# zhengyk19/vit-rpe-rope

Measured on AMD Instinct MI355X. Metric: train images/sec, CIFAR-10 ViT d=192 L=6 H=6, higher is better.
Workload: dtype bf16; 1 GPU; CIFAR-10-shaped 32x32 patch4 ViT d=192 L=6 H=6, --pos_encoding rope-axial theta=100, bf16, full train step (fwd+CE+bwd+AdamW), random-init weights; per_gpu_batch=512, global_batch=512, parallelism=dp1, hip_graph=True

## Files before the change

### include/vitpe_debug.h

```cpp
#ifndef VITPE_DEBUG_H
#define VITPE_DEBUG_H
#include "vitpe.h"
#ifdef __cplusplus
extern "C" {
#endif

int vitpe_selftest_mma(int dtype, const void* A, const void* Bt, const void* Brow, float* C_row,
                       float* C_tr, vitpe_stream_t stream);

int vitpe_debug_wgrad_census(int dtype, const vitpe_wgrad_problem* problems, int nprob, unsigned long long* census,
                             vitpe_stream_t stream);
int vitpe_debug_attn_census(const void* xn, const void* wqkv, void* out, const float* cos, const float* sin,
                            int B, unsigned long long* census, vitpe_stream_t stream);
int vitpe_debug_attn32_census(const void* xn, const void* wqkv_wide, void* out, const float* cos, const float* sin,
                              int B, unsigned long long* census, vitpe_stream_t stream);
int vitpe_debug_tail2_census(const void* attn_out, const void* x_in, const void* Wp_packed, const float* bp,
                             const float* gamma, const float* beta, void* x_mid, float* mean2, float* rstd2,
                             void* xn_out, const void* W1_packed, const float* b1, const void* W2_packed,
                             const float* b2, void* gp_out, void* h_out, void* out, float* mean_out, float* rstd_out,
                             int M, int HID, unsigned long long* census, vitpe_stream_t stream);
int vitpe_debug_set_gemm2d_mt(int mt);
int vitpe_debug_set_wgrad_wide(int on);
int vitpe_debug_read_bw(const void* src, long long bytes, int depth, int workgroups, unsigned* sink, vitpe_stream_t stream);
#ifdef __cplusplus
}
#endif
#endif
```

### vit-rpe-rope_amd/csrc/attn.hip

```cpp
#include "attn_common.h"
#include <stdlib.h>
#include <type_traits>

namespace vitpe {

template <typename T, typename C, int KM, int NTH = 384>
VITPE_DEV void stage_tokens(const AttnArgs& a, int b, T* xs, T* hbuf, int hbuf_elems, float* s_tab, float* s_coef,
                            int tid, int nthreads, bool stage_tables) {
  constexpr int CHN = CH<T>::n;
  constexpr int DCH = C::LDX / CHN;
  constexpr int D = C::DD;
  const int N = C::ntok(a);
  const T* xg = reinterpret_cast<const T*>(a.xn) + (size_t)b * N * D;
  const Chunk16 zero = {0u, 0u, 0u, 0u};
  constexpr int TOTAL = C::NP * DCH;
  constexpr int ITERS = (TOTAL + NTH - 1) / NTH;
  Chunk16 v[ITERS];
#pragma unroll
  for (int it = 0; it < ITERS; ++it) {
    const int q = tid + it * nthreads, row = q / DCH, cc = q % DCH;
    v[it] = zero;
    if (q < TOTAL && row < N && cc * CHN < D) v[it] = *reinterpret_cast<const Chunk16*>(xg + (size_t)row * D + cc * CHN);
  }
  if (a.ln_gamma != nullptr) {
// ... 477 lines not shown
    Frag<T> xf[KS];
#pragma unroll
    for (int ks = 0; ks < KS; ++ks) xf[ks] = ld_frag(xrow + 16 * tt * C::LDX + 32 * ks);
    __builtin_amdgcn_sched_barrier(0);
    f32x4 acc[NT] = {z4, z4};
#pragma unroll
    for (int ks = 0; ks < KS; ++ks)
#pragma unroll
      for (int nt = 0; nt < NT; ++nt) mma(w[nt][ks], xf[ks], acc[nt]);
    __builtin_amdgcn_sched_barrier(0);
    if (KM == KM_ROPE && rope) {
      f32x4 cv, sv;
      cs_vec(16 * tt + c, 4 * g, cv, sv);
      const f32x4 x1 = acc[0], x2 = acc[1];
      acc[0] = x1 * cv - x2 * sv;
      acc[1] = x1 * sv + x2 * cv;
    }
    dst = acc_to_frag<T>(acc[0] * sc, acc[1] * sc);
    asm volatile("" : "+v"(dst.v));
  };
  Frag<T> e0, e1;
#pragma unroll
  for (int t = 0; t < 8; ++t) {
    e0.v[t] = (bf16)((t < 4 && 4 * g + t == c) ? 1.0f : 0.0f);
    e1.v[t] = (bf16)((t >= 4 && 4 * g + t - 4 == c) ? 1.0f : 0.0f);
  }
  auto transpose_pair = [&](const Frag<T>& fa, const Frag<T>* fb, Frag<T>& d0, Frag<T>& d1) {
    f32x4 a0 = z4, a1 = z4, b0 = z4, b1 = z4;
    mma(fa, e0, a0);
    mma(fa, e1, a1);
    if (fb != nullptr) { mma(*fb, e0, b0); mma(*fb, e1, b1); }
    d0 = acc_to_frag<T>(a0, b0);
    d1 = acc_to_frag<T>(a1, b1);
  };

  const float qsc = a.scale * LOG2E;
  Frag<T> vkf[MT], kf[MT];
#pragma unroll
  for (int tt = 0; tt < MT; ++tt) proj_sw(tt, false, 1.0f, vkf[tt]);
  wload(w, 1);
  __builtin_amdgcn_sched_barrier(0);
#pragma unroll
  for (int tt = 0; tt < MT; ++tt) proj_sw(tt, true, 1.0f, kf[tt]);
  wload(w, 0);
  __builtin_amdgcn_sched_barrier(0);
#pragma unroll
  for (int tt = 0; tt < MT; ++tt) {
    Frag<T> qf;
    proj_sw(tt, true, qsc, qf);
    *reinterpret_cast<bf16x8*>(qsw + tt * FRAG) = qf.v;
  }
  __syncthreads();
  if (!live) return;
  {
    const T* dog = reinterpret_cast<const T*>(a.dout) + (size_t)b * N * D + h * HD;
    Frag<T> df[MT];
#pragma unroll
    for (int tt = 0; tt < MT; ++tt) {
      const int tok = 16 * tt + c;
      bf16x4 lo = {(bf16)0.f, (bf16)0.f, (bf16)0.f, (bf16)0.f}, hi = lo;
      if (tok < N) {
        lo = *reinterpret_cast<const bf16x4*>(dog + (size_t)tok * D + 4 * g);
        hi = *reinterpret_cast<const bf16x4*>(dog + (size_t)tok * D + 16 + 4 * g);
      }
      df[tt].v = __builtin_shufflevector(lo, hi, 0, 1, 2, 3, 4, 5, 6, 7);
    }
#pragma unroll
    for (int tt = 0; tt < MT; ++tt) *reinterpret_cast<bf16x8*>(dsw + tt * FRAG) = df[tt].v;
  }
  auto qf_load = [&](int tt) { Frag<T> f; f.v = *reinterpret_cast<const bf16x8*>(qsw + tt * FRAG); return f; };
  auto dof_load = [&](int tt) { Frag<T> f; f.v = *reinterpret_cast<const bf16x8*>(dsw + tt * FRAG); return f; };
  Frag<T> ktf[NT][SC];
#pragma unroll
  for (int scx = 0; scx < SC; ++scx)
    transpose_pair(kf[2 * scx], (2 * scx + 1 < MT) ? &kf[(2 * scx + 1 < MT) ? 2 * scx + 1 : 0] : nullptr, ktf[0][scx], ktf[1][scx]);

  T* const dqg = reinterpret_cast<T*>(a.out) + (size_t)b * N * 3 * D + h * HD;
  auto store_pair = [&](T* rowp, const f32x4& o0, const f32x4& o1, bool ok) {
    uint32_t lo[2], hi[2];
#pragma unroll
    for (int w2 = 0; w2 < 2; ++w2) {
      bf16x2 pa, pb;
      pa[0] = (bf16)o0[2 * w2]; pa[1] = (bf16)o0[2 * w2 + 1];
      pb[0] = (bf16)o1[2 * w2]; pb[1] = (bf16)o1[2 * w2 + 1];
      const auto r = __builtin_amdgcn_permlane16_swap(__builtin_bit_cast(uint32_t, pa), __builtin_bit_cast(uint32_t, pb), false, false);
      lo[w2] = r[0]; hi[w2] = r[1];
    }
    const int f0 = 16 * (g & 1) + 8 * (g >> 1);
    if (ok) *reinterpret_cast<Chunk16*>(rowp + f0) = (Chunk16){lo[0], lo[1], hi[0], hi[1]};
  };

  float cacc[PDEG + 1];
#pragma unroll
  for (int k = 0; k <= PDEG; ++k) cacc[k] = 0.f;
#pragma unroll
  for (int it = 0; it < MT; ++it) {
    __builtin_amdgcn_sched_barrier(0);
    const int i = 16 * it + c;
    const Frag<T> dof = dof_load(it), qfi = qf_load(it);
    f32x4 s[MT], dp[MT];
    float m = -1e30f;
    typedef __attribute__((ext_vector_type(4))) unsigned u32x4;
    const unsigned xyi = (KM == KM_POLY) ? reinterpret_cast<const unsigned*>(s_coef + C::H * C::PBLD)[i] : 0u;
    const float* const ptab = s_coef + (a.coeff_per_head ? h : 0) * C::PBLD;
    const bool qcls = (it == 0) && (c == 0);
#pragma unroll
    for (int jt = 0; jt < MT; ++jt) {
      s[jt] = z4;
      mma(kf[jt], qfi, s[jt]);
      dp[jt] = z4;
      mma(vkf[jt], dof, dp[jt]);
      const u32x4 xyj = (KM == KM_POLY) ? *reinterpret_cast<const u32x4*>(s_coef + C::H * C::PBLD + 16 * jt + 4 * g) : (u32x4){0u, 0u, 0u, 0u};
#pragma unroll
      for (int r = 0; r < 4; ++r) {
        const int j = 16 * jt + 4 * g + r;
        float v = s[jt][r];
        if (KM == KM_RELATIVE) v += pe_bias2<C, KM>(a, s_tab, s_coef, h, i, j, N);
        if (KM == KM_POLY) {
          const float bv = ptab[__builtin_amdgcn_sad_u8(xyi, xyj[r], 0u)];
          const bool cls = qcls || (jt == 0 && r == 0 && g == 0);
          v += cls ? 0.f : bv;
        }
        if (jt == MT - 1) v = (j < N) ? v : -1e30f;
        s[jt][r] = v;
        m = fmaxf(m, v);
      }
    }
    m = xg_max(m);
    float l = 0.f;
#pragma unroll
    for (int jt = 0; jt < MT; ++jt)
#pragma unroll
      for (int r = 0; r < 4; ++r) { const float p = __builtin_amdgcn_exp2f(s[jt][r] - m); s[jt][r] = p; l += p; }
    l = xg_sum(l);
    const float inv = __builtin_amdgcn_rcpf(l);
    float dl = 0.f;
#pragma unroll
    for (int jt = 0; jt < MT; ++jt)
#pragma unroll
      for (int r = 0; r < 4; ++r) { s[jt][r] *= inv; dl += s[jt][r] * dp[jt][r]; }
    dl = xg_sum(dl);
    if (g == 0) { lse_w[i] = m + __builtin_amdgcn_logf(l); del_w[i] = dl; }
    const bool qvalid = (it < MT - 1) || (i < N);
    float tacc[PDEG + 1];
#pragma unroll
    for (int k = 0; k <= PDEG; ++k) tacc[k] = 0.f;
#pragma unroll
    for (int jt = 0; jt < MT; ++jt) {
      if (KM == KM_POLY) __builtin_amdgcn_sched_barrier(0);
      const u32x4 xyj = (KM == KM_POLY) ? *reinterpret_cast<const u32x4*>(s_coef + C::H * C::PBLD + 16 * jt + 4 * g) : (u32x4){0u, 0u, 0u, 0u};
#pragma unroll
      for (int r = 0; r < 4; ++r) {
        const int j = 16 * jt + 4 * g + r;
        const bool valid = qvalid && ((jt < MT - 1) || (j < N));
        const float ds = valid ? s[jt][r] * (dp[jt][r] - dl) : 0.f;
        dp[jt][r] = ds;
        if (KM == KM_POLY) {
          const float dsk = (jt == 0 && r == 0) ? (g == 0 ? 0.f : ds) : ds;
          const float x = (float)__builtin_amdgcn_sad_u8(xyi, xyj[r], 0u);
          float pw = x;
          tacc[0] += dsk;
#pragma unroll
          for (int k = 1; k <= PDEG; ++k) { tacc[k] = fmaf(dsk, pw, tacc[k]); if (k < PDEG) pw *= x; }
        }
      }
    }
    if (KM == KM_POLY) {
      const float qm = (it == 0 && c == 0) ? 0.f : 1.f;
#pragma unroll
      for (int k = 0; k <= PDEG; ++k) {
        cacc[k] = fmaf(qm, tacc[k], cacc[k]);
        asm volatile("" : "+v"(cacc[k]));
      }
    }
    if (KM == KM_RELATIVE) {
#pragma unroll
      for (int jt = 0; jt < MT; ++jt) {
        float d0, d1;
        tile_diag_sums(dp[jt], lane, d0, d1);
        const int idx0 = 16 * (it - jt) + c + N - 1;
        if (g == 0) {
          if (idx0 >= 0 && idx0 <= 2 * N - 2) atomicAdd(&dtab_i[h * C::TABLD + idx0], d0);
          if (c >= 1 && idx0 - 16 >= 0 && idx0 - 16 <= 2 * N - 2) atomicAdd(&dtab_i[h * C::TABLD + idx0 - 16], d1);
        }
      }
    }
    f32x4 dqa[NT] = {z4, z4};
#pragma unroll
    for (int scx = 0; scx < SC; ++scx) {
      const Frag<T> bs = acc_to_frag<T>(dp[2 * scx], (2 * scx + 1 < MT) ? dp[(2 * scx + 1 < MT) ? 2 * scx + 1 : 0] : z4);
#pragma unroll
      for (int dt = 0; dt < NT; ++dt) mma(ktf[dt][scx], bs, dqa[dt]);
    }
    if (mixed) {
      const bool tok_ok = i >= 1 && i < N;
      f32x4 dph;
#pragma unroll
      for (int r = 0; r < 4; ++r) dph[r] = dqa[1][r] * (float)qfi.v[r] - dqa[0][r] * (float)qfi.v[4 + r];
      mixed_freq_grad_tile(dfreq_i, dph, i, tok_ok, 16 * it, h, C::H, P, a.grid, HD / 2, 4 * g, LN2, lane);
    }
    if (KM == KM_ROPE) {
      f32x4 cv, sv;
      cs_vec(min(i, C::NP - 1), 4 * g, cv, sv);
      const f32x4 d1 = dqa[0], d2 = dqa[1];
      dqa[0] = d1 * cv + d2 * sv;
      dqa[1] = d2 * cv - d1 * sv;
    }
    store_pair(dqg + (size_t)i * 3 * D, dqa[0] * a.scale, dqa[1] * a.scale, qvalid);
  }

  if (KM == KM_POLY) {
#pragma unroll
    for (int k = 0; k <= PDEG; ++k)
      if (k <= a.degree) {
        const float t = wave_sum(cacc[k]);
        if (lane == 0) atomicAdd(&dcoef_i[(a.coeff_per_head ? h : 0) * (C::MAXDEG + 1) + k], t);
      }
  }
  Frag<T> qtf[NT][SC], dotf[NT][SC];
  __builtin_amdgcn_sched_barrier(0);
#pragma unroll
  for (int scx = 0; scx < SC; ++scx) {
    const bool two = 2 * scx + 1 < MT;
    const Frag<T> qa = qf_load(2 * scx), qb = qf_load(two ? 2 * scx + 1 : 0);
    transpose_pair(qa, two ? &qb : nullptr, qtf[0][scx], qtf[1][scx]);
    const Frag<T> da = dof_load(2 * scx), db = dof_load(two ? 2 * scx + 1 : 0);
    transpose_pair(da, two ? &db : nullptr, dotf[0][scx], dotf[1][scx]);
  }
  __builtin_amdgcn_s_waitcnt(0xC07F);

#pragma unroll
  for (int jt = 0; jt < MT; ++jt) {
    __builtin_amdgcn_sched_barrier(0);
    const int j = 16 * jt + c;
    const bool kvalid = (jt < MT - 1) || (j < N);
    const unsigned xyk = (KM == KM_POLY) ? reinterpret_cast<const unsigned*>(s_coef + C::H * C::PBLD)[j] : 0u;
    const float* const ptab2 = s_coef + (a.coeff_per_head ? h : 0) * C::PBLD;
    const bool kcls = (jt == 0) && (c == 0);
    f32x4 p[MT], ds[MT];
#pragma unroll
    for (int it = 0; it < MT; ++it) {
      const Frag<T> dof = dof_load(it), qfi = qf_load(it);
      p[it] = z4;
      mma(qfi, kf[jt], p[it]);
      ds[it] = z4;
      mma(dof, vkf[jt], ds[it]);
      const f32x4 lse = *reinterpret_cast<const f32x4*>(&lse_w[16 * it + 4 * g]);
      const f32x4 dlv = *reinterpret_cast<const f32x4*>(&del_w[16 * it + 4 * g]);
      typedef __attribute__((ext_vector_type(4))) unsigned u32x4;
      const u32x4 xyq = (KM == KM_POLY) ? *reinterpret_cast<const u32x4*>(s_coef + C::H * C::PBLD + 16 * it + 4 * g) : (u32x4){0u, 0u, 0u, 0u};
#pragma unroll
      for (int r = 0; r < 4; ++r) {
        const int i = 16 * it + 4 * g + r;
        float sv = p[it][r];
        if (KM == KM_RELATIVE) sv += pe_bias2<C, KM>(a, s_tab, s_coef, h, i, j, N);
        if (KM == KM_POLY) {
          const float bv = ptab2[__builtin_amdgcn_sad_u8(xyk, xyq[r], 0u)];
          const bool cls = kcls || (it == 0 && r == 0 && g == 0);
          sv += cls ? 0.f : bv;
        }
        const bool valid = kvalid && ((it < MT - 1) || (i < N));
        const float pv = valid ? __builtin_amdgcn_exp2f(sv - lse[r]) : 0.f;
        p[it][r] = pv;
        ds[it][r] = pv * (ds[it][r] - dlv[r]);
      }
    }
    f32x4 dva[NT] = {z4, z4}, dka[NT] = {z4, z4};
#pragma unroll
    for (int scx = 0; scx < SC; ++scx) {
      const bool two = (2 * scx + 1 < MT);
      const Frag<T> bp = acc_to_frag<T>(p[2 * scx], two ? p[two ? 2 * scx + 1 : 0] : z4);
      const Frag<T> bs = acc_to_frag<T>(ds[2 * scx], two ? ds[two ? 2 * scx + 1 : 0] : z4);
#pragma unroll
      for (int dt = 0; dt < NT; ++dt) {
        mma(dotf[dt][scx], bp, dva[dt]);
        mma(qtf[dt][scx], bs, dka[dt]);
      }
    }
    dka[0] *= LN2; dka[1] *= LN2;
    if (mixed) {
      const bool tok_ok = j >= 1 && j < N;
      f32x4 dph;
#pragma unroll
      for (int r = 0; r < 4; ++r) dph[r] = dka[1][r] * (float)kf[jt].v[r] - dka[0][r] * (float)kf[jt].v[4 + r];
      mixed_freq_grad_tile(dfreq_i, dph, j, tok_ok, 16 * jt, h, C::H, P, a.grid, HD / 2, 4 * g, 1.0f, lane);
    }
    if (KM == KM_ROPE) {
      f32x4 cv, sv;
      cs_vec(min(j, C::NP - 1), 4 * g, cv, sv);
      const f32x4 d1 = dka[0], d2 = dka[1];
      dka[0] = d1 * cv + d2 * sv;
      dka[1] = d2 * cv - d1 * sv;
    }
    store_pair(dqg + (size_t)j * 3 * D + D, dka[0], dka[1], kvalid);
    store_pair(dqg + (size_t)j * 3 * D + 2 * D, dva[0], dva[1], kvalid);
  }

  __syncthreads();
  const int nrun = NTH * min(IPW, a.B - (int)blockIdx.x * IPW);
  if (KM == KM_RELATIVE) {
    for (int q = threadIdx.x; q < C::H * (2 * N - 1); q += nrun) {
      const int hh = q / (2 * N - 1), i = q % (2 * N - 1);
      atomicAdd(a.dtable + q, s_dtab[hh * C::TABLD + i]);
    }
  } else if (KM == KM_POLY) {
    const int nh = a.coeff_per_head ? C::H : 1;
    for (int q = threadIdx.x; q < nh * (a.degree + 1); q += nrun) {
      const int hh = q / (a.degree + 1), k = q % (a.degree + 1);
      atomicAdd(a.dcoeff + q, s_dcoef[hh * (C::MAXDEG + 1) + k]);
    }
  } else if (mixed) {
    for (int q = threadIdx.x; q < 2 * C::H * (HD / 2); q += nrun) atomicAdd(a.dfreqs + q, s_dfreq[q]);
  }
}

template <typename T, int HD, int D, int MT, int HPP, int KM, int NTOK>
__global__ __launch_bounds__(384) void attn_bwd_kernel(AttnArgs a) {
  using C = AttnCfg<T, HD, D, MT, HPP, NTOK>;
  __shared__ __attribute__((aligned(16))) T xs[C::NP * C::LDX];
  __shared__ __attribute__((aligned(16))) T hb[4 * HPP * C::HSZ];
  __shared__ __attribute__((aligned(16))) float s_tab[KM == KM_RELATIVE ? C::H * C::TABLD : 4];
  __shared__ __attribute__((aligned(16))) float s_coef[KM == KM_POLY ? C::PESZ : 4];
  __shared__ __attribute__((aligned(16))) float s_stat[HPP * 2 * C::NP];
  __shared__ float s_dtab[KM == KM_RELATIVE ? C::H * C::TABLD : 4];
  __shared__ float s_dcoef[C::H * (C::MAXDEG + 1)];
  __shared__ float s_dfreq[2 * C::H * (HD / 2)];
  constexpr int SLD = HPP * HD + Pad<T>::elems;
  __shared__ __attribute__((aligned(16))) T s_dq[3 * C::NP * SLD];

// ... 360 lines not shown
    if (a.ln_gamma != nullptr) hipLaunchKernelGGL((attn_fwd_kernel<T, HD, D, MT, KM, NTOK, IPW, true>), grid, block, 0, s, a);
    else hipLaunchKernelGGL((attn_fwd_kernel<T, HD, D, MT, KM, NTOK, IPW, false>), grid, block, 0, s, a);
  }
  VITPE_CHECK_LAUNCH();
}

template <typename T, int HD, int D, int MT, int HPP, int NTOK>
static int launch_attn2(bool bwd, const AttnArgs& a, hipStream_t s) {
  switch (a.mode) {
    case PE_RELATIVE: return launch_attn3<T, HD, D, MT, HPP, KM_RELATIVE, NTOK>(bwd, a, s);
    case PE_POLY: return launch_attn3<T, HD, D, MT, HPP, KM_POLY, NTOK>(bwd, a, s);
    case PE_ROPE_AXIAL:
    case PE_ROPE_MIXED: return launch_attn3<T, HD, D, MT, HPP, KM_ROPE, NTOK>(bwd, a, s);
    default: return launch_attn3<T, HD, D, MT, HPP, KM_PLAIN, NTOK>(bwd, a, s);
  }
}

template <typename T, int HD, int D, int MT, int HPP>
static int launch_attn(bool bwd, const AttnArgs& a, hipStream_t s) {
  if (a.N == 65) return launch_attn2<T, HD, D, MT, HPP, 65>(bwd, a, s);
  return launch_attn2<T, HD, D, MT, HPP, 0>(bwd, a, s);
}

static int dispatch_attn(bool bwd, int dtype, int D, int HD, const AttnArgs& a, hipStream_t s) {
  const int MT = (a.N + 15) / 16;
  if (HD != 32 || MT != 5) return (int)hipErrorNotSupported;
  if (dtype == 1) {
    if (D == 192) return launch_attn<bf16, 32, 192, 5, 2>(bwd, a, s);
    if (D == 96) return launch_attn<bf16, 32, 96, 5, 2>(bwd, a, s);
  } else if (dtype == 0) {
    if (D == 192) return launch_attn<float, 32, 192, 5, 1>(bwd, a, s);
    if (D == 96) return launch_attn<float, 32, 96, 5, 1>(bwd, a, s);
  }
  return (int)hipErrorNotSupported;
}

extern "C" int vitpe_fused_attention_supported(int dtype, int N, int D, int HD) {
  const int MT = (N + 15) / 16;
  return (dtype == 0 || dtype == 1) && HD == 32 && MT == 5 && (D == 192 || D == 96);
}

static int fused_fwd(int dtype, const void* x, const float* gamma, const float* beta, const float* mean,
                     const float* rstd, void* xn_out, const void* wqkv, void* out, int B, int N, int D, int HD,
                     const PeArgs& pe, hipStream_t stream) {
  VITPE_REQUIRE(x && wqkv && out && B >= 0 && N >= 2);
  VITPE_REQUIRE(pe_ok(pe, N, 0, 0));
  if (B == 0) return 0;
  AttnArgs a = attn_args(pe, B, N, 0, HD);
  a.xn = x; a.wqkv = wqkv; a.out = out;
  a.ln_gamma = gamma; a.ln_beta = beta; a.ln_mean = mean; a.ln_rstd = rstd; a.xn_out = xn_out;
  return dispatch_attn(false, dtype, D, HD, a, stream);
}

static int fused_bwd(int dtype, const void* x, const float* gamma, const float* beta, const float* mean,
                     const float* rstd, const void* wqkv, const void* dout, void* dqkv, int B, int N, int D, int HD,
                     const PeArgs& pe, float* dtable, float* dcoeff, float* dfreqs, hipStream_t stream) {
  VITPE_REQUIRE(x && wqkv && dout && dqkv && B >= 0 && N >= 2);
  VITPE_REQUIRE(pe_ok(pe, N, 0, 0));
  VITPE_REQUIRE(pe_grads_ok(pe.mode, dtable, dcoeff, dfreqs));
  if (B == 0) return 0;
  AttnArgs a = attn_args(pe, B, N, 0, HD);
  a.xn = x; a.wqkv = wqkv; a.out = dqkv; a.dout = dout;
  a.dtable = dtable; a.dcoeff = dcoeff; a.dfreqs = dfreqs;
  a.ln_gamma = gamma; a.ln_beta = beta; a.ln_mean = mean; a.ln_rstd = rstd;
  return dispatch_attn(true, dtype, D, HD, a, stream);
}

extern "C" int vitpe_fused_attention_fwd(int dtype, const void* xn, const void* wqkv, void* out, int B, int N,
                                         int D, int HD, int mode, const float* cos, const float* sin,
                                         const float* table, const float* coeff, int grid, int degree,
                                         int coeff_per_head, hipStream_t stream) {
  return fused_fwd(dtype, xn, nullptr, nullptr, nullptr, nullptr, nullptr, wqkv, out, B, N, D, HD,
                   {mode, cos, sin, table, coeff, grid, degree, coeff_per_head}, stream);
}

extern "C" int vitpe_fused_attention_fwd_ln(int dtype, const void* x, const float* gamma, const float* beta,
                                            const float* mean, const float* rstd, void* xn_out, const void* wqkv,
                                            void* out, int B, int N, int D, int HD, int mode, const float* cos,
                                            const float* sin, const float* table, const float* coeff, int grid,
                                            int degree, int coeff_per_head, hipStream_t stream) {
  VITPE_REQUIRE(gamma && beta && mean && rstd);
  return fused_fwd(dtype, x, gamma, beta, mean, rstd, xn_out, wqkv, out, B, N, D, HD,
                   {mode, cos, sin, table, coeff, grid, degree, coeff_per_head}, stream);
}

extern "C" int vitpe_fused_attention_bwd(int dtype, const void* xn, const void* wqkv, const void* dout,
                                         void* dqkv, int B, int N, int D, int HD, int mode, const float* cos,
                                         const float* sin, const float* table, const float* coeff, int grid,
                                         int degree, int coeff_per_head, float* dtable, float* dcoeff,
                                         float* dfreqs, hipStream_t stream) {
  return fused_bwd(dtype, xn, nullptr, nullptr, nullptr, nullptr, wqkv, dout, dqkv, B, N, D, HD,
                   {mode, cos, sin, table, coeff, grid, degree, coeff_per_head}, dtable, dcoeff, dfreqs, stream);
}

extern "C" int vitpe_fused_attention_bwd_ln(int dtype, const void* x, const float* gamma, const float* beta,
                                            const float* mean, const float* rstd, const void* wqkv, const void* dout,
                                            void* dqkv, int B, int N, int D, int HD, int mode, const float* cos,
                                            const float* sin, const float* table, const float* coeff, int grid,
                                            int degree, int coeff_per_head, float* dtable, float* dcoeff,
                                            float* dfreqs, hipStream_t stream) {
  VITPE_REQUIRE(gamma && beta && mean && rstd);
  return fused_bwd(dtype, x, gamma, beta, mean, rstd, wqkv, dout, dqkv, B, N, D, HD,
                   {mode, cos, sin, table, coeff, grid, degree, coeff_per_head}, dtable, dcoeff, dfreqs, stream);
}

extern "C" int vitpe_debug_attn_census(const void* xn, const void* wqkv, void* out, const float* cos, const float* sin,
                                       int B, unsigned long long* census, hipStream_t stream) {
  VITPE_REQUIRE(xn && wqkv && out && cos && sin && census && B > 0);
  AttnArgs a = attn_args({PE_ROPE_AXIAL, cos, sin, nullptr, nullptr, 8, 0, 0}, B, 65, 0, 32);
  a.xn = xn; a.wqkv = wqkv; a.out = out; a.census = census;
  hipLaunchKernelGGL((attn_fwd_kernel<bf16, 32, 192, 5, KM_ROPE, 65, 2, false, true>), dim3((B + 1) / 2), dim3(768), 0, stream, a);
  VITPE_CHECK_LAUNCH();
}
```

### vit-rpe-rope_amd/csrc/attn_common.h

```cpp
#pragma once
#include "common.h"

namespace vitpe {

struct AttnArgs {
  const void* xn;
  const void* wqkv;
  void* out;
  const void* dout;
  const float* cos;
  const float* sin;
  const float* table;
  const float* coeff;
  float* dtable;
  float* dcoeff;
  float* dfreqs;
  const void* qkv;
  int B, N, H;
  int mode, grid, degree, coeff_per_head;
  float scale;
  const float* ln_gamma;
  const float* ln_beta;
  const float* ln_mean;
  const float* ln_rstd;
  void* xn_out;
  unsigned long long* census;
  void* qkv_out;
  float* tab_slab;
  const unsigned long long* rng;
  unsigned drop_thr;
  float drop_rs;
  int cls_only;
};

struct PeArgs {
  int mode;
  const float *cos, *sin, *table, *coeff;
  int grid, degree, coeff_per_head;
};

inline bool pe_ok(const PeArgs& pe, int N, int H, int hmax) {
  if (pe.mode == PE_ROPE_AXIAL || pe.mode == PE_ROPE_MIXED) {
    if (!pe.cos || !pe.sin || pe.grid * pe.grid != N - 1) return false;
    if (pe.mode == PE_ROPE_MIXED && hmax && H > hmax) return false;
  }
  if (pe.mode == PE_RELATIVE && !pe.table) return false;
  if (pe.mode == PE_POLY && (!pe.coeff || pe.degree < 0 || pe.degree > 7 || pe.grid * pe.grid != N - 1)) return false;
  return pe.mode >= PE_NONE && pe.mode <= PE_ROPE_MIXED;
}

inline bool pe_grads_ok(int mode, const float* dtable, const float* dcoeff, const float* dfreqs) {
  if (mode == PE_RELATIVE) return dtable != nullptr;
  if (mode == PE_POLY) return dcoeff != nullptr;
  if (mode == PE_ROPE_MIXED) return dfreqs != nullptr;
  return true;
}

inline AttnArgs attn_args(const PeArgs& pe, int B, int N, int H, int HD) {
  AttnArgs a{};
  a.cos = pe.cos; a.sin = pe.sin; a.table = pe.table; a.coeff = pe.coeff;
  a.mode = pe.mode; a.grid = pe.grid; a.degree = pe.degree; a.coeff_per_head = pe.coeff_per_head;
  a.B = B; a.N = N; a.H = H;
  a.scale = 1.0f / sqrtf((float)HD);
  return a;
}

constexpr float LOG2E = 1.4426950408889634f;
constexpr float LN2 = 0.6931471805599453f;

enum { KM_PLAIN = 0, KM_RELATIVE = 1, KM_POLY = 2, KM_ROPE = 3, KM_ROPE_TABLES = 4 };

template <typename T, int HD, int D, int MT, int HPP, int NTOK>
struct AttnCfg {
  static constexpr int H = D / HD;
  static constexpr int NT = HD / 16;
  static constexpr int KS = D / 32;
  static constexpr int HC = HD / 32;
  static constexpr int NP = 16 * MT;
  static constexpr int SC = (MT + 1) / 2;
  static constexpr int VR = 32 * SC;
  static constexpr int LDX = D + (sizeof(T) == 2 ? 2 : 1) * Pad<T>::elems;
  static constexpr int LDH = HD + (sizeof(T) == 2 ? 2 : 1) * Pad<T>::elems;
  static constexpr int HSZ = VR * LDH;
  static constexpr int QSZ = NP * LDH;
  static constexpr int TABLD = 2 * NP;
// ... 133 lines not shown
```

### vit-rpe-rope_amd/csrc/tail2.hip

```cpp
#include "common.h"
#include <type_traits>
#include <stdlib.h>

#ifndef T2_RB
#define T2_RB 6
#endif
#ifndef T2_NV
#define T2_NV 8
#endif

namespace vitpe {

struct Tail2Args {
  const void* a;
  const void* xin;
  const void* wp;
  const float* bp;
  const float* gamma;
  const float* beta;
  const void* w1;
  const float* b1;
  const void* w2;
  const float* b2;
  void* xmid;
// ... 536 lines not shown
    o0[2 * w2 + 1] = __uint_as_float(r[0] & 0xffff0000u);
    o1[2 * w2] = __uint_as_float(r[1] << 16);
    o1[2 * w2 + 1] = __uint_as_float(r[1] & 0xffff0000u);
  }
}

VITPE_DEV void t2_unpack_pair_f16(const Chunk16& v, f32x4& o0, f32x4& o1) {
#pragma unroll
  for (int w2 = 0; w2 < 2; ++w2) {
    const auto r = __builtin_amdgcn_permlane16_swap(v[w2], v[2 + w2], false, false);
    const uint32_t ra = r[0], rb = r[1];
    o0[2 * w2] = (float)__builtin_bit_cast(_Float16, (unsigned short)(ra & 0xffffu));
    o0[2 * w2 + 1] = (float)__builtin_bit_cast(_Float16, (unsigned short)(ra >> 16));
    o1[2 * w2] = (float)__builtin_bit_cast(_Float16, (unsigned short)(rb & 0xffffu));
    o1[2 * w2 + 1] = (float)__builtin_bit_cast(_Float16, (unsigned short)(rb >> 16));
  }
}

VITPE_DEV void t2_load_rows(bool even, const bf16* line, int step, bf16x4 (&v)[T2_NT]) {
  Chunk16 l[6];
#pragma unroll
  for (int m = 0; m < 3; ++m) {
    l[2 * m] = *reinterpret_cast<const Chunk16*>(line + 64 * m);
    l[2 * m + 1] = *reinterpret_cast<const Chunk16*>(line + step + 64 * m);
  }
#pragma unroll
  for (int m = 0; m < 3; ++m) {
    Chunk16 h[2];
    t2_line_xchg(even, l[2 * m], l[2 * m + 1], h[0], h[1]);
#pragma unroll
    for (int s = 0; s < 2; ++s) {
      const auto r0 = __builtin_amdgcn_permlane16_swap(h[s][0], h[s][2], false, false);
      const auto r1 = __builtin_amdgcn_permlane16_swap(h[s][1], h[s][3], false, false);
      v[4 * m + 2 * s] = __builtin_bit_cast(bf16x4, (uint2){r0[0], r1[0]});
      v[4 * m + 2 * s + 1] = __builtin_bit_cast(bf16x4, (uint2){r0[1], r1[1]});
    }
  }
}

template <int CTRL> VITPE_DEV float t2_dppc(float v) {
  return __builtin_bit_cast(float, __builtin_amdgcn_update_dpp(0, __builtin_bit_cast(int, v), CTRL, 0xf, 0xf, true));
}
VITPE_DEV float t2_colsum8(const float (&t)[8], int c) {
  const bool b3 = (c & 8) != 0, b2 = (c & 4) != 0, b1 = (c & 2) != 0;
  float u[4], w[2];
#pragma unroll
  for (int k = 0; k < 4; ++k) u[k] = (b3 ? t[4 + k] : t[k]) + t2_dppc<0x128>(b3 ? t[k] : t[4 + k]);
#pragma unroll
  for (int k = 0; k < 2; ++k) w[k] = (b2 ? u[2 + k] : u[k]) + t2_dppc<0x141>(b2 ? u[k] : u[2 + k]);
  const float x = (b1 ? w[1] : w[0]) + t2_dppc<0x4E>(b1 ? w[0] : w[1]);
  return x + t2_dppc<0xB1>(x);
}

VITPE_DEV void t2_ln_backward(f32x4 (&acc)[T2_NT], const bf16* xline, const bf16* rline, int lstep, float mean, float rstd,
                              const float* sGam, float* sAcc, int c, int g, float valid, const T2Row& orow) {
  constexpr int D = T2_D, NT = T2_NT;
  const bool even = (c & 1) == 0;
  bf16x4 xmv[NT];
  t2_load_rows(even, xline, lstep, xmv);
  const float invD = 1.0f / (float)D;
  float s1 = 0.f, s2 = 0.f;
#pragma unroll
  for (int nt = 0; nt < NT; ++nt) {
    __builtin_amdgcn_sched_barrier(0);
    const f32x4 gam = *reinterpret_cast<const f32x4*>(sGam + 16 * nt + 4 * g);
    float tot[8];
#pragma unroll
    for (int r = 0; r < 4; ++r) {
      const float xhat = ((float)xmv[nt][r] - mean) * rstd;
      const float dxn = acc[nt][r];
      tot[r] = dxn * xhat * valid;
      tot[4 + r] = dxn * valid;
      const float gy = dxn * gam[r];
      s1 += gy;
      s2 = fmaf(gy, xhat, s2);
    }
    const float sel = t2_colsum8(tot, c);
    asm volatile("" : "+v"(s1), "+v"(s2));
    if (!(c & 1)) atomicAdd(&sAcc[(c < 8 ? 0 : D - 4) + 16 * nt + 4 * g + (c >> 1)], sel);
  }
  const float m1 = t2_xg_sum(s1) * invD, m2 = t2_xg_sum(s2) * invD;
  bf16x4 rv[NT];
  t2_load_rows(even, rline, lstep, rv);
#pragma unroll
  for (int nt = 0; nt < NT; ++nt) {
    __builtin_amdgcn_sched_barrier(0);
    uint2 xw = __builtin_bit_cast(uint2, xmv[nt]);
    asm volatile("" : "+v"(xw.x), "+v"(xw.y));
    const bf16x4 xb = __builtin_bit_cast(bf16x4, xw);
    const f32x4 gam = *reinterpret_cast<const f32x4*>(sGam + 16 * nt + 4 * g);
#pragma unroll
    for (int r = 0; r < 4; ++r) {
      const float xhat = ((float)xb[r] - mean) * rstd;
      const float gy = acc[nt][r] * gam[r];
      acc[nt][r] = to_f32(from_f32<bf16>(fmaf(rstd, gy - m1 - xhat * m2, (float)rv[nt][r])));
    }
  }
#pragma unroll
  for (int nt = 0; nt < NT; nt += 2) t2_store_pair<T2_AUX_ROW>(orow, nt, g, acc[nt], acc[nt + 1]);
}

VITPE_DEV void t2_flush_colsums(float* sAcc, int* sFin, int nactive, int lane, float* dgamma, float* dbeta) {
  asm volatile("s_waitcnt lgkmcnt(0)" ::: "memory");
  int fin = 0;
  if (lane == 0) fin = atomicAdd(sFin, 1);
  fin = __builtin_amdgcn_readfirstlane(fin);
  if (fin == nactive - 1) {
    for (int i = lane; i < T2_D; i += 64) {
      atomicAdd(dgamma + i, __hip_atomic_load(&sAcc[i], __ATOMIC_RELAXED, __HIP_MEMORY_SCOPE_WORKGROUP));
      atomicAdd(dbeta + i, __hip_atomic_load(&sAcc[T2_D + i], __ATOMIC_RELAXED, __HIP_MEMORY_SCOPE_WORKGROUP));
    }
  }
}

template <bool PRE>
__global__ __launch_bounds__(T2_THREADS) void block_tail2_bwd_kernel(Tail2BwdArgs a) {
  using T = bf16;
  constexpr int D = T2_D, NT = T2_NT, KS = T2_KS;
  __shared__ __attribute__((aligned(16))) T sW[3 * T2_SLABF * 512];
  __shared__ __attribute__((aligned(16))) float sGam[T2_D], sGam1[PRE ? T2_D : 4];
  __shared__ float sAcc[2 * T2_D], sAcc1[PRE ? 2 * T2_D : 4];
  __shared__ int sReady[T2_NFLAG], sDone[T2_NFLAG], sFin;

  const int lane = threadIdx.x & 63, c = lane & 15, g = lane >> 4;
  const int wave = __builtin_amdgcn_readfirstlane(threadIdx.x >> 6);
  const int HID = a.HID, nchunk = HID / T2_CH, nsub = 2 * nchunk;
  const int nkc = PRE ? a.K1 / 64 : 0, Q = (nkc + 1) / 2, QB = nkc / 2;
  const int ntiles = (a.M + 15) / 16, base = ntiles / (int)gridDim.x, rem = ntiles % (int)gridDim.x;
  const int tile0 = (int)blockIdx.x * base + min((int)blockIdx.x, rem), ntile_wg = base + ((int)blockIdx.x < rem ? 1 : 0);
  const bool active = wave < ntile_wg;
  const int row = 16 * (tile0 + wave) + c;
  const int rowc = min(row, a.M - 1);
  const float valid = row < a.M ? 1.0f : 0.0f;

  if (threadIdx.x < T2_NFLAG) { sReady[threadIdx.x] = 0; sDone[threadIdx.x] = 0; }
  if (threadIdx.x == 0) sFin = 0;
  for (int i = threadIdx.x; i < 2 * D; i += T2_THREADS) { sAcc[i] = 0.f; if (PRE) sAcc1[i] = 0.f; }
  for (int i = threadIdx.x; i < D; i += T2_THREADS) { sGam[i] = a.gamma[i]; if (PRE) sGam1[i] = a.gamma1[i]; }

  auto dma1 = [&](const T* src_frag, int dst_frag) {
    __builtin_amdgcn_global_load_lds((const __attribute__((address_space(1))) void*)(src_frag + lane * 8),
                                     (__attribute__((address_space(3))) void*)(sW + dst_frag * 512), 16, 0, 0);
  };
  if (wave >= T2_WAVES) {
    __builtin_amdgcn_s_setprio(T2_LOADER_PRIO);
    const bool is1 = wave == T2_WAVES;
    const int nq = is1 ? Q : QB, njobs = nq + nchunk;
    const int half = is1 ? 0 : T2_HALF;
// ... 57 lines not shown
    asm volatile("s_waitcnt lgkmcnt(0)" ::: "memory");
    if (lane == 0) atomicAdd(&sDone[k], 1);
  };
  auto slab_ptr = [&](int gs) { return sW + ((gs + 2) % 3) * T2_SLABF * 512 + lane * 8; };

  Frag<T> bf[KS];
  const bool even = (c & 1) == 0;
  const int lrow = min(row & ~1, a.M - 1), lnext = min((row & ~1) + 1, a.M - 1) - lrow;
  const T* const dql = PRE ? reinterpret_cast<const T*>(a.dqkv) + (size_t)lrow * a.K1 + 32 * (c & 1) + 8 * g : nullptr;
  const int dqstep = PRE ? lnext * a.K1 : 0;
  const int lpiece = 32 * (c & 1) + 16 * (g & 1) + 8 * (g >> 1);
  const size_t lrowD = (size_t)lrow * D + lpiece;
  Frag<T> bqa[4], bqb[4];
  auto ld_qlines = [&](Frag<T> (&f)[4], int q) {
#pragma unroll
    for (int i = 0; i < 4; ++i) f[i] = ld_frag(dql + (i & 1) * dqstep + 64 * min(2 * q + (i >> 1), nkc - 1));
  };
  if (active) {
    if (PRE) {
      ld_qlines(bqa, 0);
    } else {
      bf16x4 dv[NT];
      t2_load_rows(even, reinterpret_cast<const T*>(a.dy) + lrowD, lnext * D, dv);
#pragma unroll
      for (int ks = 0; ks < KS; ++ks) bf[ks].v = __builtin_shufflevector(dv[2 * ks], dv[2 * ks + 1], 0, 1, 2, 3, 4, 5, 6, 7);
    }
  }
  __builtin_amdgcn_s_waitcnt(0x0070);
  asm volatile("s_barrier" ::: "memory");
  if (!active) return;

  if (PRE) {
    f32x4 acc[NT];
#pragma unroll
    for (int nt = 0; nt < NT; ++nt) acc[nt] = (f32x4){0.f, 0.f, 0.f, 0.f};
    const int nks = a.K1 / 32;
    auto qslab = [&](int q, Frag<T> (&cur)[4], Frag<T> (&nxt)[4]) {
      if (q + 1 < Q) ld_qlines(nxt, q + 1);
      t2_lines_to_frags(even, cur[0], cur[1]);
      t2_lines_to_frags(even, cur[2], cur[3]);
      wait_ready(q);
      const T* wb = slab_ptr(q);
      t2_gemm<NT, 2, 8>(wb, cur, acc);
      if (4 * q + 2 < nks) t2_gemm<NT, 2, 8>(wb + T2_HALF * 512, cur + 2, acc);
      signal_done(q + 1);
    };
    for (int q = 0; q < Q; q += 2) {
      qslab(q, bqa, bqb);
      if (q + 1 < Q) qslab(q + 1, bqb, bqa);
    }
    t2_ln_backward(acc, reinterpret_cast<const T*>(a.x1) + lrowD, reinterpret_cast<const T*>(a.dres1) + lrowD, lnext * D,
                   a.mean1[rowc], a.rstd1[rowc], sGam1, sAcc1, c, g, valid, t2_row(const_cast<void*>(a.dy), 16 * tile0, rowc, D));
#pragma unroll
    for (int ks = 0; ks < KS; ++ks) bf[ks] = acc_to_frag<T>(acc[2 * ks], acc[2 * ks + 1]);
  }

  const int lstep = lnext * HID;
  const T* const gpl = reinterpret_cast<const T*>(a.gp) + (size_t)lrow * HID + lpiece;
  const T2Row dul = t2_row(a.du, 16 * tile0, lrow, HID) + lpiece;
  Chunk16 gq[2];
  gq[0] = *reinterpret_cast<const Chunk16*>(gpl);
  gq[1] = *reinterpret_cast<const Chunk16*>(gpl + lstep);
  Chunk16 godd;
  t2_u32x4 duh;
  f32x4 acc2[NT];
#pragma unroll
  for (int nt = 0; nt < NT; ++nt) acc2[nt] = (f32x4){0.f, 0.f, 0.f, 0.f};
  f32x4 aX[2], aY[2];
  Frag<T> hP, hQ;
  const f32x4 z4 = {0.f, 0.f, 0.f, 0.f};
  auto gstage_even = [&](const f32x4 (&a1c)[2], int p, Frag<T>& hnew) {
    f32x4 g0, g1, d0, d1;
    Chunk16 cur;
    t2_line_xchg(even, gq[0], gq[1], cur, godd);
    if (p + 1 < nchunk) {
      gq[0] = *reinterpret_cast<const Chunk16*>(gpl + 64 * (p + 1));
      gq[1] = *reinterpret_cast<const Chunk16*>(gpl + lstep + 64 * (p + 1));
    }
    t2_unpack_pair_f16(cur, g0, g1);
#pragma unroll
    for (int r = 0; r < 4; ++r) { d0[r] = a1c[0][r] * g0[r]; d1[r] = a1c[1][r] * g1[r]; }
    duh = t2_pack_pair(d0, d1);
    asm volatile("" : "+v"(duh));
    hnew = acc_to_frag<T>(d0, d1);
  };
  auto gstage_odd = [&](const f32x4 (&a1c)[2], int p, Frag<T>& hnew) {
    f32x4 g0, g1, d0, d1;
    t2_unpack_pair_f16(godd, g0, g1);
#pragma unroll
    for (int r = 0; r < 4; ++r) { d0[r] = a1c[0][r] * g0[r]; d1[r] = a1c[1][r] * g1[r]; }
    t2_u32x4 l0, l1;
    t2_line_xchg(even, duh, t2_pack_pair(d0, d1), l0, l1);
    __builtin_amdgcn_raw_buffer_store_b128(l0, dul.rsrc, dul.off + 128 * p, 0, T2_AUX_HID);
    __builtin_amdgcn_raw_buffer_store_b128(l1, dul.rsrc, dul.off + 2 * lstep + 128 * p, 0, T2_AUX_HID);
    hnew = acc_to_frag<T>(d0, d1);
  };
  constexpr int NVB = 3, RB = T2_RB;

  wait_ready(Q);
  {
    const T* wb = slab_ptr(Q);
    aX[0] = z4; aX[1] = z4;
    t2_step<true, false, 0, RB>(wb, wb, bf, aX, hQ, acc2, [&]() {});
    aY[0] = z4; aY[1] = z4;
    t2_step<true, false, 2 * NVB, RB>(wb + 2 * KS * 512, wb, bf, aY, hQ, acc2, [&]() { gstage_even(aX, 0, hP); });
    signal_done(Q + 1);
  }
  for (int p = 1; p < nchunk; ++p) {
    wait_ready(Q + p);
    const T* wb = slab_ptr(Q + p);
    const T* w2b = wb + T2_HALF * 512;
    aX[0] = z4; aX[1] = z4;
    t2_step<true, true, NVB, RB>(wb, w2b, bf, aX, hP, acc2, [&]() { gstage_odd(aY, p - 1, hQ); });
    aY[0] = z4; aY[1] = z4;
    t2_step<true, true, NVB, RB>(wb + 2 * KS * 512, w2b + NT * 512, bf, aY, hQ, acc2, [&]() { gstage_even(aX, p, hP); });
    signal_done(Q + p + 1);
  }
  wait_ready(Q + nchunk);
  {
    const T* w2b = slab_ptr(Q + nchunk) + T2_HALF * 512;
    t2_step<false, true, 2 * NVB, RB>(w2b, w2b, bf, aX, hP, acc2, [&]() { gstage_odd(aY, nchunk - 1, hQ); });
    t2_step<false, true, 0, RB>(w2b, w2b + NT * 512, bf, aX, hQ, acc2, [&]() {});
    signal_done(Q + nchunk + 1);
  }
  t2_ln_backward(acc2, reinterpret_cast<const T*>(a.xmid) + lrowD, reinterpret_cast<const T*>(a.dy) + lrowD, lnext * D,
                 a.mean2[rowc], a.rstd2[rowc], sGam, sAcc, c, g, valid, t2_row(a.dxmid, 16 * tile0, rowc, D));
#pragma unroll
  for (int ks = 0; ks < KS; ++ks) bf[ks] = acc_to_frag<T>(acc2[2 * ks], acc2[2 * ks + 1]);
  f32x4 accA[NT];
#pragma unroll
  for (int nt = 0; nt < NT; ++nt) accA[nt] = z4;
  wait_ready(Q + nchunk + 1);
  t2_gemm<NT, KS, 12>(sW + lane * 8, bf, accA);
  {
    const T2Row dar = t2_row(a.da, 16 * tile0, rowc, D);
#pragma unroll
    for (int nt = 0; nt < NT; nt += 2) t2_store_pair<T2_AUX_ROW>(dar, nt, g, accA[nt], accA[nt + 1]);
  }
  asm volatile("s_waitcnt lgkmcnt(0)" ::: "memory");
  int fin = 0;
  if (lane == 0) fin = atomicAdd(&sFin, 1);
  fin = __builtin_amdgcn_readfirstlane(fin);
  if (fin == ntile_wg - 1) {
    for (int i = lane; i < D; i += 64) {
      atomicAdd(a.dgamma + i, __hip_atomic_load(&sAcc[i], __ATOMIC_RELAXED, __HIP_MEMORY_SCOPE_WORKGROUP));
      atomicAdd(a.dbeta + i, __hip_atomic_load(&sAcc[D + i], __ATOMIC_RELAXED, __HIP_MEMORY_SCOPE_WORKGROUP));
      if (PRE) {
        atomicAdd(a.dgamma1 + i, __hip_atomic_load(&sAcc1[i], __ATOMIC_RELAXED, __HIP_MEMORY_SCOPE_WORKGROUP));
        atomicAdd(a.dbeta1 + i, __hip_atomic_load(&sAcc1[D + i], __ATOMIC_RELAXED, __HIP_MEMORY_SCOPE_WORKGROUP));
      }
    }
  }
}

struct LnBwd2Args {
  const void* dy;
  const void* wt;
  const void* x;
  const float* mean;
  const float* rstd;
  const float* gamma;
  const void* dres;
  void* dx;
  float* dgamma;
  float* dbeta;
  int M, K;
};

__global__ __launch_bounds__(T2_THREADS) void ln_bwd2_kernel(LnBwd2Args a) {
  using T = bf16;
  constexpr int D = T2_D, NT = T2_NT, KS = T2_KS, SLF = NT * KS;
  __shared__ __attribute__((aligned(16))) T sW[2 * SLF * 512];
  __shared__ __attribute__((aligned(16))) float sGam[T2_D];
  __shared__ float sAcc[2 * T2_D];
  __shared__ int sReady[T2_NFLAG], sDone[T2_NFLAG], sFin;

  const int lane = threadIdx.x & 63, c = lane & 15, g = lane >> 4;
  const int wave = __builtin_amdgcn_readfirstlane(threadIdx.x >> 6);
  const int K = a.K, nslab = K / D;
// ... 226 lines not shown
```

Baseline: 375,600 images/sec.

## Skip zero-gradient query tiles in attention backward and reuse residual fragments

```diff
diff --git a/include/vitpe_debug.h b/include/vitpe_debug.h
--- a/include/vitpe_debug.h
+++ b/include/vitpe_debug.h
@@ -21,6 +21,7 @@
                              int M, int HID, unsigned long long* census, vitpe_stream_t stream);
 int vitpe_debug_set_gemm2d_mt(int mt);
 int vitpe_debug_set_wgrad_wide(int on);
+int vitpe_debug_set_attn_bwd_skip(int on);
 int vitpe_debug_read_bw(const void* src, long long bytes, int depth, int workgroups, unsigned* sink, vitpe_stream_t stream);
 #ifdef __cplusplus
 }
diff --git a/vit-rpe-rope_amd/csrc/attn.hip b/vit-rpe-rope_amd/csrc/attn.hip
--- a/vit-rpe-rope_amd/csrc/attn.hip
+++ b/vit-rpe-rope_amd/csrc/attn.hip
@@ -553,6 +553,7 @@
   }
   __syncthreads();
   if (!live) return;
+  bool nz[MT];
   {
     const T* dog = reinterpret_cast<const T*>(a.dout) + (size_t)b * N * D + h * HD;
     Frag<T> df[MT];
@@ -567,8 +568,14 @@
       df[tt].v = __builtin_shufflevector(lo, hi, 0, 1, 2, 3, 4, 5, 6, 7);
     }
 #pragma unroll
-    for (int tt = 0; tt < MT; ++tt) *reinterpret_cast<bf16x8*>(dsw + tt * FRAG) = df[tt].v;
-  }
+    for (int tt = 0; tt < MT; ++tt) {
+      *reinterpret_cast<bf16x8*>(dsw + tt * FRAG) = df[tt].v;
+      const Chunk16 dw = __builtin_bit_cast(Chunk16, df[tt].v);
+      const uint32_t mag = (dw[0] | dw[1] | dw[2] | dw[3]) & 0x7fff7fffu;
+      nz[tt] = __builtin_amdgcn_ballot_w64(mag != 0u) != 0ull || a.bwd_noskip != 0;
+    }
+  }
+  constexpr int RV = NTOK != 0 ? NTOK - 16 * (MT - 1) : 4;
   auto qf_load = [&](int tt) { Frag<T> f; f.v = *reinterpret_cast<const bf16x8*>(qsw + tt * FRAG); return f; };
   auto dof_load = [&](int tt) { Frag<T> f; f.v = *reinterpret_cast<const bf16x8*>(dsw + tt * FRAG); return f; };
   Frag<T> ktf[NT][SC];
@@ -598,6 +605,10 @@
   for (int it = 0; it < MT; ++it) {
     __builtin_amdgcn_sched_barrier(0);
     const int i = 16 * it + c;
+    if (!nz[it]) {
+      store_pair(dqg + (size_t)i * 3 * D, z4, z4, (it < MT - 1) || (i < N));
+      continue;
+    }
     const Frag<T> dof = dof_load(it), qfi = qf_load(it);
     f32x4 s[MT], dp[MT];
     float m = -1e30f;
@@ -614,6 +625,7 @@
       const u32x4 xyj = (KM == KM_POLY) ? *reinterpret_cast<const u32x4*>(s_coef + C::H * C::PBLD + 16 * jt + 4 * g) : (u32x4){0u, 0u, 0u, 0u};
 #pragma unroll
       for (int r = 0; r < 4; ++r) {
+        if (jt == MT - 1 && r >= RV) continue;
         const int j = 16 * jt + 4 * g + r;
         float v = s[jt][r];
         if (KM == KM_RELATIVE) v += pe_bias2<C, KM>(a, s_tab, s_coef, h, i, j, N);
@@ -632,14 +644,20 @@
 #pragma unroll
     for (int jt = 0; jt < MT; ++jt)
 #pragma unroll
-      for (int r = 0; r < 4; ++r) { const float p = __builtin_amdgcn_exp2f(s[jt][r] - m); s[jt][r] = p; l += p; }
+      for (int r = 0; r < 4; ++r) {
+        if (jt == MT - 1 && r >= RV) { s[jt][r] = 0.f; continue; }
+        const float p = __builtin_amdgcn_exp2f(s[jt][r] - m); s[jt][r] = p; l += p;
+      }
     l = xg_sum(l);
     const float inv = __builtin_amdgcn_rcpf(l);
     float dl = 0.f;
 #pragma unroll
     for (int jt = 0; jt < MT; ++jt)
 #pragma unroll
-      for (int r = 0; r < 4; ++r) { s[jt][r] *= inv; dl += s[jt][r] * dp[jt][r]; }
+      for (int r = 0; r < 4; ++r) {
+        if (jt == MT - 1 && r >= RV) continue;
+        s[jt][r] *= inv; dl += s[jt][r] * dp[jt][r];
+      }
     dl = xg_sum(dl);
     if (g == 0) { lse_w[i] = m + __builtin_amdgcn_logf(l); del_w[i] = dl; }
     const bool qvalid = (it < MT - 1) || (i < N);
@@ -652,6 +670,7 @@
       const u32x4 xyj = (KM == KM_POLY) ? *reinterpret_cast<const u32x4*>(s_coef + C::H * C::PBLD + 16 * jt + 4 * g) : (u32x4){0u, 0u, 0u, 0u};
 #pragma unroll
       for (int r = 0; r < 4; ++r) {
+        if (jt == MT - 1 && r >= RV) { dp[jt][r] = 0.f; continue; }
         const int j = 16 * jt + 4 * g + r;
         const bool valid = qvalid && ((jt < MT - 1) || (j < N));
         const float ds = valid ? s[jt][r] * (dp[jt][r] - dl) : 0.f;
@@ -738,22 +757,21 @@
     const unsigned xyk = (KM == KM_POLY) ? reinterpret_cast<const unsigned*>(s_coef + C::H * C::PBLD)[j] : 0u;
     const float* const ptab2 = s_coef + (a.coeff_per_head ? h : 0) * C::PBLD;
     const bool kcls = (jt == 0) && (c == 0);
-    f32x4 p[MT], ds[MT];
-#pragma unroll
-    for (int it = 0; it < MT; ++it) {
+    auto pds_tile = [&](int it, f32x4& pt, f32x4& dst) {
       const Frag<T> dof = dof_load(it), qfi = qf_load(it);
-      p[it] = z4;
-      mma(qfi, kf[jt], p[it]);
-      ds[it] = z4;
-      mma(dof, vkf[jt], ds[it]);
+      pt = z4;
+      mma(qfi, kf[jt], pt);
+      dst = z4;
+      mma(dof, vkf[jt], dst);
       const f32x4 lse = *reinterpret_cast<const f32x4*>(&lse_w[16 * it + 4 * g]);
       const f32x4 dlv = *reinterpret_cast<const f32x4*>(&del_w[16 * it + 4 * g]);
       typedef __attribute__((ext_vector_type(4))) unsigned u32x4;
       const u32x4 xyq = (KM == KM_POLY) ? *reinterpret_cast<const u32x4*>(s_coef + C::H * C::PBLD + 16 * it + 4 * g) : (u32x4){0u, 0u, 0u, 0u};
 #pragma unroll
       for (int r = 0; r < 4; ++r) {
+        if (it == MT - 1 && r >= RV) { pt[r] = 0.f; dst[r] = 0.f; continue; }
         const int i = 16 * it + 4 * g + r;
-        float sv = p[it][r];
+        float sv = pt[r];
         if (KM == KM_RELATIVE) sv += pe_bias2<C, KM>(a, s_tab, s_coef, h, i, j, N);
         if (KM == KM_POLY) {
           const float bv = ptab2[__builtin_amdgcn_sad_u8(xyk, xyq[r], 0u)];
@@ -762,20 +780,43 @@
         }
         const bool valid = kvalid && ((it < MT - 1) || (i < N));
         const float pv = valid ? __builtin_amdgcn_exp2f(sv - lse[r]) : 0.f;
-        p[it][r] = pv;
-        ds[it][r] = pv * (ds[it][r] - dlv[r]);
-      }
-    }
+        pt[r] = pv;
+        dst[r] = pv * (dst[r] - dlv[r]);
+      }
+    };
     f32x4 dva[NT] = {z4, z4}, dka[NT] = {z4, z4};
-#pragma unroll
-    for (int scx = 0; scx < SC; ++scx) {
-      const bool two = (2 * scx + 1 < MT);
-      const Frag<T> bp = acc_to_frag<T>(p[2 * scx], two ? p[two ? 2 * scx + 1 : 0] : z4);
-      const Frag<T> bs = acc_to_frag<T>(ds[2 * scx], two ? ds[two ? 2 * scx + 1 : 0] : z4);
+    auto pair_mma = [&](int scx, const f32x4& p0, const f32x4& p1, const f32x4& ds0, const f32x4& ds1) {
+      const Frag<T> bp = acc_to_frag<T>(p0, p1);
+      const Frag<T> bs = acc_to_frag<T>(ds0, ds1);
 #pragma unroll
       for (int dt = 0; dt < NT; ++dt) {
         mma(dotf[dt][scx], bp, dva[dt]);
         mma(qtf[dt][scx], bs, dka[dt]);
+      }
+    };
+    bool dense = true;
+#pragma unroll
+    for (int it = 0; it < MT; ++it) dense = dense && nz[it];
+    if (dense) {
+      f32x4 p[MT], ds[MT];
+#pragma unroll
+      for (int it = 0; it < MT; ++it) pds_tile(it, p[it], ds[it]);
+#pragma unroll
+      for (int scx = 0; scx < SC; ++scx) {
+        const bool two = (2 * scx + 1 < MT);
+        pair_mma(scx, p[2 * scx], two ? p[two ? 2 * scx + 1 : 0] : z4, ds[2 * scx], two ? ds[two ? 2 * scx + 1 : 0] : z4);
+      }
+    } else {
+#pragma unroll
+      for (int scx = 0; scx < SC; ++scx) {
+        const bool two = (2 * scx + 1 < MT);
+        const int ia = 2 * scx, ib = two ? 2 * scx + 1 : 0;
+        if (nz[ia] || (two && nz[ib])) {
+          f32x4 p0 = z4, p1 = z4, ds0 = z4, ds1 = z4;
+          if (nz[ia]) pds_tile(ia, p0, ds0);
+          if (two && nz[ib]) pds_tile(ib, p1, ds1);
+          pair_mma(scx, p0, p1, ds0, ds1);
+        }
       }
     }
     dka[0] *= LN2; dka[1] *= LN2;
@@ -1242,6 +1283,9 @@
   return dispatch_attn(false, dtype, D, HD, a, stream);
 }
 
+static bool g_bwd_skip = true;
+extern "C" int vitpe_debug_set_attn_bwd_skip(int on) { g_bwd_skip = on != 0; return 0; }
+
 static int fused_bwd(int dtype, const void* x, const float* gamma, const float* beta, const float* mean,
                      const float* rstd, const void* wqkv, const void* dout, void* dqkv, int B, int N, int D, int HD,
                      const PeArgs& pe, float* dtable, float* dcoeff, float* dfreqs, hipStream_t stream) {
@@ -1253,6 +1297,7 @@
   a.xn = x; a.wqkv = wqkv; a.out = dqkv; a.dout = dout;
   a.dtable = dtable; a.dcoeff = dcoeff; a.dfreqs = dfreqs;
   a.ln_gamma = gamma; a.ln_beta = beta; a.ln_mean = mean; a.ln_rstd = rstd;
+  a.bwd_noskip = g_bwd_skip ? 0 : 1;
   return dispatch_attn(true, dtype, D, HD, a, stream);
 }
 
diff --git a/vit-rpe-rope_amd/csrc/attn_common.h b/vit-rpe-rope_amd/csrc/attn_common.h
--- a/vit-rpe-rope_amd/csrc/attn_common.h
+++ b/vit-rpe-rope_amd/csrc/attn_common.h
@@ -31,6 +31,7 @@
   unsigned drop_thr;
   float drop_rs;
   int cls_only;
+  int bwd_noskip;
 };
 
 struct PeArgs {
diff --git a/vit-rpe-rope_amd/csrc/tail2.hip b/vit-rpe-rope_amd/csrc/tail2.hip
--- a/vit-rpe-rope_amd/csrc/tail2.hip
+++ b/vit-rpe-rope_amd/csrc/tail2.hip
@@ -612,8 +612,10 @@
   return x + t2_dppc<0xB1>(x);
 }
 
+template <bool RFRAG = false>
 VITPE_DEV void t2_ln_backward(f32x4 (&acc)[T2_NT], const bf16* xline, const bf16* rline, int lstep, float mean, float rstd,
-                              const float* sGam, float* sAcc, int c, int g, float valid, const T2Row& orow) {
+                              const float* sGam, float* sAcc, int c, int g, float valid, const T2Row& orow,
+                              const Frag<bf16>* rfrag = nullptr) {
   constexpr int D = T2_D, NT = T2_NT;
   const bool even = (c & 1) == 0;
   bf16x4 xmv[NT];
@@ -641,7 +643,7 @@
   }
   const float m1 = t2_xg_sum(s1) * invD, m2 = t2_xg_sum(s2) * invD;
   bf16x4 rv[NT];
-  t2_load_rows(even, rline, lstep, rv);
+  if constexpr (!RFRAG) t2_load_rows(even, rline, lstep, rv);
 #pragma unroll
   for (int nt = 0; nt < NT; ++nt) {
     __builtin_amdgcn_sched_barrier(0);
@@ -653,7 +655,8 @@
     for (int r = 0; r < 4; ++r) {
       const float xhat = ((float)xb[r] - mean) * rstd;
       const float gy = acc[nt][r] * gam[r];
-      acc[nt][r] = to_f32(from_f32<bf16>(fmaf(rstd, gy - m1 - xhat * m2, (float)rv[nt][r])));
+      const float res = RFRAG ? (float)rfrag[nt >> 1].v[4 * (nt & 1) + r] : (float)rv[nt][r];
+      acc[nt][r] = to_f32(from_f32<bf16>(fmaf(rstd, gy - m1 - xhat * m2, res)));
     }
   }
 #pragma unroll
@@ -817,7 +820,10 @@
     t2_ln_backward(acc, reinterpret_cast<const T*>(a.x1) + lrowD, reinterpret_cast<const T*>(a.dres1) + lrowD, lnext * D,
                    a.mean1[rowc], a.rstd1[rowc], sGam1, sAcc1, c, g, valid, t2_row(const_cast<void*>(a.dy), 16 * tile0, rowc, D));
 #pragma unroll
-    for (int ks = 0; ks < KS; ++ks) bf[ks] = acc_to_frag<T>(acc[2 * ks], acc[2 * ks + 1]);
+    for (int ks = 0; ks < KS; ++ks) {
+      bf[ks] = acc_to_frag<T>(acc[2 * ks], acc[2 * ks + 1]);
+      asm volatile("" : "+v"(bf[ks].v));
+    }
   }
 
   const int lstep = lnext * HID;
@@ -888,8 +894,8 @@
     t2_step<false, true, 0, RB>(w2b, w2b + NT * 512, bf, aX, hQ, acc2, [&]() {});
     signal_done(Q + nchunk + 1);
   }
-  t2_ln_backward(acc2, reinterpret_cast<const T*>(a.xmid) + lrowD, reinterpret_cast<const T*>(a.dy) + lrowD, lnext * D,
-                 a.mean2[rowc], a.rstd2[rowc], sGam, sAcc, c, g, valid, t2_row(a.dxmid, 16 * tile0, rowc, D));
+  t2_ln_backward<true>(acc2, reinterpret_cast<const T*>(a.xmid) + lrowD, nullptr, lnext * D,
+                       a.mean2[rowc], a.rstd2[rowc], sGam, sAcc, c, g, valid, t2_row(a.dxmid, 16 * tile0, rowc, D), bf);
 #pragma unroll
   for (int ks = 0; ks < KS; ++ks) bf[ks] = acc_to_frag<T>(acc2[2 * ks], acc2[2 * ks + 1]);
   f32x4 accA[NT];
```

Result: no change. 375,100 images/sec (-0.1%).
